# zju3dv/LoFTR

Hardware: AMD Instinct MI355X
Metric: image-pairs/sec @640x480 indoor-ds (higher is better)
Workload: dtype f32; 1 GPU; batch=8 640x480 synthetic grayscale pairs per GPU, indoor_ds dual-softmax (BASELINE configs[1]), full LoFTR.forward = ResNet-FPN backbone (HIP implicit-GEMM / patch convolutions incl. the 7x7 stem) + HIP matching path; weights=seeded random init (no checkpoint on the box), conf_matrix_materialised=True, match_type=dual_softmax, global_batch=8, parallelism=dp1 (pairs sharded; RCCL all-gather of match counts)

## Files before the change

loftr_amd/csrc/common.h:

```cpp
#pragma once
#include <hip/hip_runtime.h>
#include <stdint.h>
#include <stddef.h>
#include "../../include/loftr_hip.h"

typedef float f32x16 __attribute__((ext_vector_type(16)));
typedef float f32x4 __attribute__((ext_vector_type(4)));
typedef float f32x2 __attribute__((ext_vector_type(2)));

#define LOFTR_NEG_INF (-1e9f)

#define LOFTR_CHECK_ARG(cond) do { if (!(cond)) return LOFTR_ERR_BAD_ARG; } while (0)
#define LOFTR_CHECK_LAUNCH() do { if (hipGetLastError() != hipSuccess) return LOFTR_ERR_LAUNCH; } while (0)

#ifdef __HIP_DEVICE_COMPILE__
#define LOFTR_NO_PACKED_FP32 __attribute__((target("no-packed-fp32-ops")))
#else
#define LOFTR_NO_PACKED_FP32
#endif

__host__ __device__ static inline int ceil_div(int a, int b) { return (a + b - 1) / b; }
static inline size_t align_up(size_t x, size_t a) { return (x + a - 1) / a * a; }

enum LoftrTimedKernel {
  LOFTR_T_SCORE_STATS = 0,
  LOFTR_T_SCORE_CONF = 1,
  LOFTR_T_PROJ = 2,
  LOFTR_T_LINEAR = 3,
  LOFTR_T_LINEAR_LN = 4,
  LOFTR_T_KV = 5,
  LOFTR_T_ATTN_APPLY = 6,
  LOFTR_T_ATTN_SMALL = 7,
  LOFTR_T_GATHER = 8,
  LOFTR_T_OT_STORE = 9,
  LOFTR_T_CONV = 10,
  LOFTR_T_CONV3 = 11,
  LOFTR_T_CONV3W = 12,
  LOFTR_T_ENCODER_X = 13,
  LOFTR_T_FINE_PAIR = 14,
  LOFTR_T_COUNT = 15
};
enum LoftrDebugKey {
  LOFTR_DBG_ENCODER_SCHEDULE = 0,
  LOFTR_DBG_CONV_PERSIST_CAP,
  LOFTR_DBG_WGRAD_CHUNK,
  LOFTR_DBG_REDUCE_TALL,
  LOFTR_DBG_PCT_GRID,
  LOFTR_DBG_PCT_SKIP,
  LOFTR_DBG_PCT_QUOTA,
  LOFTR_DBG_CONV_DUO,
  LOFTR_DBG_CONV_PATCH,
  LOFTR_DBG_CONV_REM,
  LOFTR_DBG_FINE_WAVES,
  LOFTR_DBG_COUNT
};
int loftr_debug_value(int key);
extern unsigned g_loftr_timing_mask;
extern int g_loftr_range_check;
void loftr_timing_mark(int id, hipStream_t st, bool end);
struct TimedLaunch {
  int id; hipStream_t st; bool on;
  TimedLaunch(int id_, hipStream_t st_) : id(id_), st(st_), on((g_loftr_timing_mask >> id_) & 1u) {
    if (on) loftr_timing_mark(id, st, false);
  }
  ~TimedLaunch() { if (on) loftr_timing_mark(id, st, true); }
};

constexpr int NUM_XCD = 8;
static inline unsigned xcd_grid(int tiles_m, int tiles_n) { return (unsigned)(NUM_XCD * ceil_div(tiles_m, NUM_XCD) * tiles_n); }
__device__ __forceinline__ bool xcd_tile(int tiles_m, int tiles_n, int& tile_m, int& tile_n) {
  const int id = blockIdx.x, xcd = id % NUM_XCD, slot = id / NUM_XCD;
  const int chunk = ceil_div(tiles_m, NUM_XCD);
  tile_n = slot % tiles_n;
  const int local = slot / tiles_n;
  tile_m = xcd * chunk + local;
  return local < chunk && tile_m < tiles_m;
}

struct WsAlloc {
  char* base; size_t cap; size_t off;
  WsAlloc(void* p, size_t bytes) : base((char*)p), cap(bytes), off(0) {}
  template <typename T> T* take(size_t n) {
    off = align_up(off, 256);
    T* r = (T*)(base + off);
    off += n * sizeof(T);
    return r;
  }
  bool ok() const { return off <= cap; }
};

__device__ __forceinline__ float wave_sum(float v) {
#pragma unroll
  for (int o = 32; o >= 1; o >>= 1) v += __shfl_xor(v, o, 64);
  return v;
}
__device__ __forceinline__ float wave_max(float v) {
#pragma unroll
  for (int o = 32; o >= 1; o >>= 1) v = fmaxf(v, __shfl_xor(v, o, 64));
  return v;
}
#define LOFTR_DPP(v_, ctrl_) __int_as_float(__builtin_amdgcn_update_dpp(0, __float_as_int(v_), ctrl_, 0xF, 0xF, true))
#define LOFTR_DPPI(v_, ctrl_) __builtin_amdgcn_update_dpp(0, v_, ctrl_, 0xF, 0xF, true)
__device__ __forceinline__ float half_sum(float v) {
  v += LOFTR_DPP(v, 0xB1);
  v += LOFTR_DPP(v, 0x4E);
  v += LOFTR_DPP(v, 0x141);
  v += LOFTR_DPP(v, 0x140);
  const auto r = __builtin_amdgcn_permlane16_swap(__float_as_int(v), __float_as_int(v), false, false);
  return __int_as_float(r[0]) + __int_as_float(r[1]);
}
__device__ __forceinline__ float half_max(float v) {
  v = fmaxf(v, LOFTR_DPP(v, 0xB1));
  v = fmaxf(v, LOFTR_DPP(v, 0x4E));
  v = fmaxf(v, LOFTR_DPP(v, 0x141));
  v = fmaxf(v, LOFTR_DPP(v, 0x140));
  const auto r = __builtin_amdgcn_permlane16_swap(__float_as_int(v), __float_as_int(v), false, false);
  return fmaxf(__int_as_float(r[0]), __int_as_float(r[1]));
}
__device__ __forceinline__ int half_min_i32(int v) {
  v = min(v, LOFTR_DPPI(v, 0xB1));
  v = min(v, LOFTR_DPPI(v, 0x4E));
  v = min(v, LOFTR_DPPI(v, 0x141));
  v = min(v, LOFTR_DPPI(v, 0x140));
  const auto r = __builtin_amdgcn_permlane16_swap(v, v, false, false);
  return min((int)r[0], (int)r[1]);
}
__device__ __forceinline__ void half_sum16(f32x16& v) {
#pragma unroll
  for (int r = 0; r < 16; ++r) v[r] += LOFTR_DPP(v[r], 0xB1);
#pragma unroll
  for (int r = 0; r < 16; ++r) v[r] += LOFTR_DPP(v[r], 0x4E);
#pragma unroll
  for (int r = 0; r < 16; ++r) v[r] += LOFTR_DPP(v[r], 0x141);
#pragma unroll
  for (int r = 0; r < 16; ++r) v[r] += LOFTR_DPP(v[r], 0x140);
#pragma unroll
// ... 30 lines not shown
```

loftr_amd/csrc/conv.hip:

```cpp
#include "gemm.h"
#include "conv_prepared.h"
#include <stdlib.h>

namespace {

using CfgD = GemmCfg<256, 128, 4, 2, 3>;

struct ConvArgs {
  ASrc a;
  const sp_t* w; int K;
  const float* bias;
  const float* wscale;
  const float* x_inv;
  const sp_t* residual;
  sp_t* y_sp;
  float* y_f32;
  int M, Cout, Coutp;
  int act;
  const sp_t* up;
  int Hl, Wl;
  float sy, sx;
};

template <typename Cfg, bool FULL>
__device__ __forceinline__ void conv_epilogue(const ConvArgs& p, f32x16 (&acc)[Cfg::TM][Cfg::TN], int m0, int n0) {
  const EpiLane<Cfg> e;
  const sp_t* rs = p.residual ? p.residual + (long)m0 * p.Coutp + n0 : nullptr;
  sp_t* os = p.y_sp ? p.y_sp + (long)m0 * p.Coutp + n0 : nullptr;
  float* of = p.y_f32 ? p.y_f32 + (long)m0 * p.Cout + n0 : nullptr;
#pragma unroll
  for (int j = 0; j < Cfg::TN; ++j) {
    const int col = n0 + e.lcol + j * 32;
    const bool creal = col < p.Cout;
    const bool cpad = col < p.Coutp;
    const float b = (p.bias && creal) ? p.bias[col] : 0.f;
    const float wsc = (creal ? p.wscale[col] : 1.f) * (p.x_inv ? *p.x_inv : 1.f);
#pragma unroll
    for (int i = 0; i < Cfg::TM; ++i) {
      f32x16 v = acc[i][j] * wsc;
      if (rs) {
        uint32_t w[16];
#pragma unroll
        for (int r = 0; r < 16; ++r) {
          const int trow = e.lrow + e.rr(i, r);
          const bool ok = (FULL || m0 + trow < p.M) && cpad;
          w[r] = ok ? rs[(unsigned)(trow * p.Coutp + e.spcol + j * 32)] : 0u;
        }
#pragma unroll
        for (int r = 0; r < 16; ++r) v[r] += sp_value(w[r], e.odd);
      }
#pragma unroll
      for (int r = 0; r < 16; ++r) {
        float x = v[r] + b;
        if (p.act == 1) x = fmaxf(x, 0.f);
        if (p.act == 2) x = x > 0.f ? x : 0.01f * x;
        v[r] = creal ? x : 0.f;
      }
      if (of) {
#pragma unroll
        for (int r = 0; r < 16; ++r) {
          const int trow = e.lrow + e.rr(i, r);
          if ((FULL || m0 + trow < p.M) && creal) of[(unsigned)(trow * p.Cout + e.lcol + j * 32)] = v[r];
        }
      }
      if (os) {
        uint32_t w[16];
        sp_words16(v, e.odd, w);
#pragma unroll
        for (int r = 0; r < 16; ++r) {
          const int trow = e.lrow + e.rr(i, r);
          if ((FULL || m0 + trow < p.M) && cpad) os[(unsigned)(trow * p.Coutp + e.spcol + j * 32)] = w[r];
        }
      }
    }
  }
}

template <typename Cfg>
__device__ __forceinline__ void conv_epilogue_up(const ConvArgs& p, f32x16 (&acc)[Cfg::TM][Cfg::TN], int m0, int n0,
                                                 float* lds) {
  constexpr int LD = Cfg::BN + 4;
  static_assert(Cfg::BM * LD <= Cfg::LDS_FLOATS, "accumulator tile does not fit the operand ring");
  const EpiLane<Cfg> e;
  __syncthreads();
  const float xinv = p.x_inv ? *p.x_inv : 1.f;
#pragma unroll
  for (int j = 0; j < Cfg::TN; ++j) {
    const int col = n0 + e.lcol + j * 32;
    const float wsc = (col < p.Cout ? p.wscale[col] : 1.f) * xinv;
#pragma unroll
    for (int i = 0; i < Cfg::TM; ++i)
#pragma unroll
      for (int r = 0; r < 16; ++r) lds[(e.lrow + e.rr(i, r)) * LD + e.lcol + j * 32] = acc[i][j][r] * wsc;
  }
  __syncthreads();
  const int Wo = 2 * p.Wl, Ho = 2 * p.Hl;
  constexpr int OCTS = Cfg::BN / 8;
  for (int it = threadIdx.x; it < Cfg::BM * OCTS; it += Cfg::THREADS) {
    const int row = it / OCTS, oct = it - row * OCTS;
    const int pix = m0 + row, col0 = n0 + oct * 8;
    if (pix >= p.M || col0 >= p.Coutp) continue;
    const int t = pix / Wo, x = pix - t * Wo;
    const int bb = t / Ho, y = t - bb * Ho;
    const float fy = p.sy * (float)y, fx = p.sx * (float)x;
    const int y0 = (int)fy, x0 = (int)fx;
    const int dy = y0 < p.Hl - 1 ? p.Wl * p.Coutp : 0, dx = x0 < p.Wl - 1 ? p.Coutp : 0;
    const float ly = fy - (float)y0, lx = fx - (float)x0;
    const float hy = 1.f - ly, hx = 1.f - lx;
    const int off = sp_octet_off(col0 >> 3);
    const sp_t* s00 = p.up + (unsigned)(((bb * p.Hl + y0) * p.Wl + x0) * p.Coutp + off);
    const sp_t* src[4] = {s00, s00 + dx, s00 + dy, s00 + dy + dx};
    u32x4 hi[4], lo[4];
#pragma unroll
    for (int k = 0; k < 4; ++k) {
      hi[k] = *reinterpret_cast<const u32x4*>(src[k]);
      lo[k] = *reinterpret_cast<const u32x4*>(src[k] + 16);
    }
    float v[4][8], o[8];
#pragma unroll
    for (int k = 0; k < 4; ++k) sp_unpack8(hi[k], lo[k], v[k]);
    const f32x4 a0 = *reinterpret_cast<const f32x4*>(&lds[row * LD + oct * 8]);
    const f32x4 a1 = *reinterpret_cast<const f32x4*>(&lds[row * LD + oct * 8 + 4]);
#pragma unroll
    for (int c = 0; c < 8; ++c)
      o[c] = col0 + c < p.Cout
                 ? (c < 4 ? a0[c] : a1[c - 4]) + (hy * (hx * v[0][c] + lx * v[1][c]) + ly * (hx * v[2][c] + lx * v[3][c]))
                 : 0.f;
    u32x4 oh, ol;
    sp_pack8(o, oh, ol);
    sp_t* dst = p.y_sp + (unsigned)(pix * p.Coutp + off);
    *reinterpret_cast<u32x4*>(dst) = oh;
    *reinterpret_cast<u32x4*>(dst + 16) = ol;
  }
}

template <typename Cfg, bool UP>
__global__ __launch_bounds__(Cfg::THREADS, 2) void conv_kernel(ConvArgs p) {
  __shared__ __attribute__((aligned(16))) float lds[Cfg::LDS_FLOATS];
  int tm, tn;
  if (!xcd_tile(ceil_div(p.M, Cfg::BM), ceil_div(p.Coutp, Cfg::BN), tm, tn)) return;
  const int m0 = tm * Cfg::BM, n0 = tn * Cfg::BN;
  f32x16 acc[Cfg::TM][Cfg::TN];
  gemm_mainloop<Cfg, true>(p.a, p.w, p.K, p.M, p.Cout, p.K, m0, n0, lds, acc, p.Coutp);
  if constexpr (UP) conv_epilogue_up<Cfg>(p, acc, m0, n0, lds);
  else if (m0 + Cfg::BM <= p.M) conv_epilogue<Cfg, true>(p, acc, m0, n0);
  else conv_epilogue<Cfg, false>(p, acc, m0, n0);
}

namespace c3 {
constexpr int TY = 8, TX = 32, PW = TX + 2, PH = TY + 2, PROWS = PW * PH;
constexpr int PSLOTS = 43, PQ = 6;
constexpr int PATCH_BYTES = PSLOTS * 1024, BTILE_BYTES = 128 * 128;
constexpr int NB = 4;
constexpr int LDS_BYTES = 2 * PATCH_BYTES + NB * BTILE_BYTES + 1024;
using Cfg = GemmCfg<256, 128, 4, 2, 3>;
}

struct Conv3Args {
  const sp_t* x; int B, H, W, Cp, Cin;
  const sp_t* w; int K;
  const float* bias; const float* wscale; const float* x_inv; const sp_t* residual; sp_t* y_sp; float* y_f32;
  int Cout, Coutp, act;
  const sp_t* zeros;
  int tiles_x, tiles_y;
  float* pbuf;
};

__global__ __launch_bounds__(512, 2) void conv3x3_kernel(Conv3Args p) {
  using namespace c3;
  typedef __attribute__((address_space(3))) void* lds_ptr_t;
  typedef const __attribute__((address_space(1))) void* gbl_ptr_t;
  __shared__ __attribute__((aligned(16))) char lds[LDS_BYTES];
  char* const patch_base = lds;
  char* const bring_base = lds + 2 * PATCH_BYTES;
  char* const scratch = lds + 2 * PATCH_BYTES + NB * BTILE_BYTES;

  const int tid = threadIdx.x, lane = tid & 63, wave = tid >> 6;
  const int wm = wave & 3, wn = wave >> 2;
  const int rsub = lane >> 3, slot = lane & 7;

  const int tiles_m = p.B * p.tiles_y * p.tiles_x, tiles_n = ceil_div(p.Coutp, 128);
  const int chunk_m = ceil_div(tiles_m, NUM_XCD), nvirt = NUM_XCD * chunk_m * tiles_n;
  int vid = blockIdx.x;
  int nb = 0, ny0 = 0, nx0 = 0, nn0 = 0;
  bool have = false;
#define C3_NEXT_TILE()                                                                                      \
  {                                                                                                         \
    have = false;                                                                                           \
    for (; vid < nvirt; vid += gridDim.x) {                                                                 \
      const int xcd__ = vid % NUM_XCD, slot__ = vid / NUM_XCD;                                              \
      const int local__ = slot__ / tiles_n, tm__ = xcd__ * chunk_m + local__;                               \
      if (local__ < chunk_m && tm__ < tiles_m) {                                                            \
        nb = tm__ / (p.tiles_y * p.tiles_x);                                                                \
        const int trem__ = tm__ - nb * (p.tiles_y * p.tiles_x);                                             \
        ny0 = (trem__ / p.tiles_x) * TY; nx0 = (trem__ % p.tiles_x) * TX; nn0 = (slot__ % tiles_n) * 128;   \
        have = true;                                                                                        \
        break;                                                                                              \
      }                                                                                                     \
    }                                                                                                       \
  }
  C3_NEXT_TILE()
  if (!have) return;

  int poff[PQ];
  int boff[2];
#define C3_DMA_OFFSETS()                                                                                    \
  {                                                                                                         \
    _Pragma("unroll") for (int q = 0; q < PQ; ++q) {                                                        \
      const int s = q * 8 + wave, r = s * 8 + rsub;                                                         \
      const int py = r / PW, px = r - py * PW;                                                              \
      const int gy = ny0 - 1 + py, gx = nx0 - 1 + px;                                                       \
      const bool in = s < PSLOTS && r < PROWS && (unsigned)gy < (unsigned)p.H && (unsigned)gx < (unsigned)p.W; \
      poff[q] = in ? ((nb * p.H + gy) * p.W + gx) * p.Cp + ((slot ^ ((r >> 1) & 7)) << 2) : -1;             \
    }                                                                                                       \
    _Pragma("unroll") for (int q = 0; q < 2; ++q) {                                                         \
      const int r = (q * 8 + wave) * 8 + rsub;                                                              \
      boff[q] = min(nn0 + r, p.Cout - 1) * p.K + ((slot ^ ((r >> 1) & 7)) << 2);                            \
    }                                                                                                       \
  }
  C3_DMA_OFFSETS()
// ... 230 lines not shown
  const int co = blockIdx.x;
  float scale = 1.f, shift = 0.f;
  if (bn_w) {
    scale = bn_w[co] / sqrtf(bn_v[co] + eps);
    shift = bn_b[co] - bn_m[co] * scale;
  }
  float m = 0.f;
  for (int t = threadIdx.x; t < Cin * KH * KW; t += 256) {
    const int c = t % Cin, tap = t / Cin;
    m = fmaxf(m, fabsf(w[co * s_co + c * s_ci + (tap / KW) * s_ky + (tap % KW) * s_kx] * scale));
  }
  __shared__ float red[4];
  m = wave_max(m);
  if ((threadIdx.x & 63) == 0) red[threadIdx.x >> 6] = m;
  __syncthreads();
  if (threadIdx.x == 0) {
    float inv;
    (void)sp_row_scale(fmaxf(fmaxf(red[0], red[1]), fmaxf(red[2], red[3])), &inv);
    bias[co] = shift;
    wscale[co] = inv;
  }
}

__global__ __launch_bounds__(256) void conv_prep_kernel(const float* __restrict__ w, const float* __restrict__ bn_w,
                                                        const float* __restrict__ bn_b, const float* __restrict__ bn_m,
                                                        const float* __restrict__ bn_v, float eps, int Cin, int Cp,
                                                        int KH, int KW, long s_co, long s_ci, long s_ky, long s_kx,
                                                        sp_t* __restrict__ wsp, const float* __restrict__ wscale) {
  const int co = blockIdx.y;
  const int K = KH * KW * Cp;
  float scale = 1.f;
  if (bn_w) scale = bn_w[co] / sqrtf(bn_v[co] + eps);
  const float up = 1.f / wscale[co];
  const int grp = blockIdx.x * 8 + (threadIdx.x >> 5);
  if (grp * 32 >= K) return;
  const int col = grp * 32 + (threadIdx.x & 31);
  const int tap = col / Cp, c = col - tap * Cp;
  float v = 0.f;
  if (c < Cin) v = (w[co * s_co + c * s_ci + (tap / KW) * s_ky + (tap % KW) * s_kx] * scale) * up;
  sp_store(wsp + (long)co * K, col, v, true);
}

__global__ __launch_bounds__(256) void upsample_add_kernel(const sp_t* __restrict__ low, const sp_t* __restrict__ lat,
                                                           sp_t* __restrict__ out, int Hl, int Wl, int Cp, long nitems) {
  const long item = (long)blockIdx.x * 256 + threadIdx.x;
  if (item >= nitems) return;
  const int octs = Cp >> 3;
  const long pix = item / octs;
  const int oct = (int)(item - pix * octs);
  const int Ho = 2 * Hl, Wo = 2 * Wl;
  const int x = (int)(pix % Wo), y = (int)((pix / Wo) % Ho);
  const long b = pix / ((long)Wo * Ho);
  const float sy = Ho > 1 ? (float)(Hl - 1) / (float)(Ho - 1) : 0.f, sx = Wo > 1 ? (float)(Wl - 1) / (float)(Wo - 1) : 0.f;
  const float fy = sy * (float)y, fx = sx * (float)x;
  const int y0 = (int)fy, x0 = (int)fx;
  const int y1 = y0 + (y0 < Hl - 1 ? 1 : 0), x1 = x0 + (x0 < Wl - 1 ? 1 : 0);
  const float ly = fy - (float)y0, lx = fx - (float)x0;
  const float hy = 1.f - ly, hx = 1.f - lx;
  const int off = sp_octet_off(oct);
  const sp_t* src[5] = {low + ((b * Hl + y0) * Wl + x0) * Cp + off, low + ((b * Hl + y0) * Wl + x1) * Cp + off,
                        low + ((b * Hl + y1) * Wl + x0) * Cp + off, low + ((b * Hl + y1) * Wl + x1) * Cp + off,
                        lat + pix * Cp + off};
  u32x4 hi[5], lo[5];
#pragma unroll
  for (int t = 0; t < 5; ++t) {
    hi[t] = *reinterpret_cast<const u32x4*>(src[t]);
    lo[t] = *reinterpret_cast<const u32x4*>(src[t] + 16);
  }
  float v[5][8];
#pragma unroll
  for (int t = 0; t < 5; ++t) sp_unpack8(hi[t], lo[t], v[t]);
  float r[8];
#pragma unroll
  for (int e = 0; e < 8; ++e)
    r[e] = v[4][e] + (hy * (hx * v[0][e] + lx * v[1][e]) + ly * (hx * v[2][e] + lx * v[3][e]));
  u32x4 oh, ol;
  sp_pack8(r, oh, ol);
  sp_t* o = out + pix * Cp + off;
  *reinterpret_cast<u32x4*>(o) = oh;
  *reinterpret_cast<u32x4*>(o + 16) = ol;
}

constexpr int STEM_TY = 8, STEM_TX = 32;
__global__ __launch_bounds__(256) void stem_conv_kernel(const float* __restrict__ x, long sxb, long sxh, long sxw,
                                                        int H, int W, const float* __restrict__ w, long s_co, long s_ky,
                                                        long s_kx, const float* __restrict__ bn_w,
                                                        const float* __restrict__ bn_b, const float* __restrict__ bn_m,
                                                        const float* __restrict__ bn_v, float eps, int C0, int Ho, int Wo,
                                                        sp_t* __restrict__ y) {
  constexpr int IH = 2 * STEM_TY + 5, IW = 2 * STEM_TX + 5;
  __shared__ float tile[IH][IW + 3];
  const int b = blockIdx.z, oy0 = blockIdx.y * STEM_TY, ox0 = blockIdx.x * STEM_TX;
  const float* xb = x + (long)b * sxb;
  for (int e = threadIdx.x; e < IH * IW; e += 256) {
    const int r = e / IW, c = e - r * IW;
    const int iy = 2 * oy0 - 3 + r, ix = 2 * ox0 - 3 + c;
    tile[r][c] = ((unsigned)iy < (unsigned)H && (unsigned)ix < (unsigned)W) ? xb[iy * sxh + ix * sxw] : 0.f;
  }
  const int ch = threadIdx.x & 127, slot = threadIdx.x >> 7;
  float wr[49];
  float scale = 1.f, shift = 0.f;
  if (ch < C0) {
    if (bn_w) { scale = bn_w[ch] / sqrtf(bn_v[ch] + eps); shift = bn_b[ch] - bn_m[ch] * scale; }
#pragma unroll
    for (int t = 0; t < 49; ++t) wr[t] = w[ch * s_co + (t / 7) * s_ky + (t % 7) * s_kx] * scale;
  } else {
#pragma unroll
    for (int t = 0; t < 49; ++t) wr[t] = 0.f;
  }
  __syncthreads();
  const int Cp = (C0 + 31) / 32 * 32;
  for (int q = slot; q < STEM_TY * STEM_TX / 4; q += 2) {
    const int py = q / (STEM_TX / 4), px = (q - py * (STEM_TX / 4)) * 4;
    float acc[4] = {shift, shift, shift, shift};
#pragma unroll
    for (int ky = 0; ky < 7; ++ky) {
      float row[13];
#pragma unroll
      for (int c = 0; c < 13; ++c) row[c] = tile[2 * py + ky][2 * px + c];
#pragma unroll
      for (int kx = 0; kx < 7; ++kx)
#pragma unroll
        for (int e = 0; e < 4; ++e) acc[e] += row[2 * e + kx] * wr[ky * 7 + kx];
    }
    const int oy = oy0 + py;
#pragma unroll
    for (int e = 0; e < 4; ++e) {
      const int ox = ox0 + px + e;
      const float v = fmaxf(acc[e], 0.f);
      const bool ok = oy < Ho && ox < Wo && ch < Cp;
      const uint32_t word = sp_word(ch < C0 ? v : 0.f, ch & 1);
      if (ok) y[(((long)b * Ho + oy) * Wo + ox) * Cp + sp_index(ch)] = word;
    }
  }
}

__global__ void sp_to_f32_kernel(const sp_t* __restrict__ src, float* __restrict__ dst, long rows, int C, int Cp) {
  const long row = blockIdx.x;
  for (int c = threadIdx.x; c < Cp; c += blockDim.x) {
    const float v = sp_value(src[row * Cp + sp_index(c)], c & 1);
    if (c < C) dst[row * C + c] = v;
  }
}

}

extern "C" size_t loftr_conv_workspace_bytes(int Cin, int Cout, int KH, int KW) {
  if (Cin <= 0 || Cout <= 0 || KH <= 0 || KW <= 0) return 0;
  return align_up((size_t)Cout * KH * KW * ceil32(Cin) * 4, 256) + 2 * align_up((size_t)Cout * 4, 256) + 2048;
}

static unsigned persistent_grid(unsigned nvirt) {
  const int cap = loftr_debug_value(LOFTR_DBG_CONV_PERSIST_CAP);
  const int forced = cap >= NUM_XCD ? cap / NUM_XCD * NUM_XCD : -1;
  int cus = forced;
  if (cus < 0) {
    static int per_dev[64];
    int dev = 0, n = 0;
    if (hipGetDevice(&dev) != hipSuccess || dev < 0 || dev >= 64) return nvirt;
    if (per_dev[dev] == 0) {
      if (hipDeviceGetAttribute(&n, hipDeviceAttributeMultiprocessorCount, dev) != hipSuccess) return nvirt;
      per_dev[dev] = n / NUM_XCD * NUM_XCD;
    }
    cus = per_dev[dev];
  }
  return cus > 0 && nvirt > (unsigned)cus ? (unsigned)cus : nvirt;
}

template <int RT>
__global__ __launch_bounds__(256) void conv_rem_gather_kernel(const float* __restrict__ pbuf, long npix, int H, int W, int R, int c0, int Coutp,
                                                              const float* __restrict__ bias, const sp_t* __restrict__ residual, int act,
                                                              sp_t* __restrict__ y_sp) {
  const long pix = (long)blockIdx.x * 256 + threadIdx.x;
  if (pix >= npix) return;
  const int x = (int)(pix % W), y = (int)((pix / W) % H);
  float v[8];
#pragma unroll
  for (int c = 0; c < 8; ++c) v[c] = 0.f;
  const float* pp = pbuf + pix * (9 * R);
#pragma unroll
  for (int ky = 0; ky < 3; ++ky)
#pragma unroll
    for (int kx = 0; kx < 3; ++kx) {
      const int yy = y + ky - 1, xx = x + kx - 1;
      if ((unsigned)yy < (unsigned)H && (unsigned)xx < (unsigned)W) {
        const float* q = pp + ((long)(ky - 1) * W + (kx - 1)) * (9 * R) + (ky * 3 + kx) * R;
        if (RT == 4) {
          const f32x4 t = *reinterpret_cast<const f32x4*>(q);
          v[0] += t[0]; v[1] += t[1]; v[2] += t[2]; v[3] += t[3];
        } else {
#pragma unroll
          for (int c = 0; c < 7; ++c) if (c < R) v[c] += q[c];
        }
      }
    }
  sp_t* row = y_sp + pix * Coutp + c0;
  float rv[8];
#pragma unroll
  for (int c = 0; c < 8; ++c) rv[c] = 0.f;
  if (residual) {
    const sp_t* rr = residual + pix * Coutp + c0;
    const u32x4 hi = *reinterpret_cast<const u32x4*>(rr), lo = *reinterpret_cast<const u32x4*>(rr + 16);
    sp_unpack8(hi, lo, rv);
  }
  const float slope = act == 1 ? 0.f : act == 2 ? 0.01f : 1.f;
  float o[8];
#pragma unroll
  for (int c = 0; c < 8; ++c) {
    const float t = v[c] + ((bias && c < R) ? bias[c0 + c] : 0.f) + rv[c];
    o[c] = c < R ? fmaxf(t, slope * t) : 0.f;
  }
  u32x4 oh, ol;
  sp_pack8(o, oh, ol);
  const u32x4 z = {0u, 0u, 0u, 0u};
  u32x4* dst = reinterpret_cast<u32x4*>(row);
  dst[0] = oh; dst[1] = z; dst[2] = z; dst[3] = z; dst[4] = ol; dst[5] = z; dst[6] = z; dst[7] = z;
}


static int conv_prepare(const float* weight, const long* weight_strides, int Cin, int Cout, int KH, int KW,
                        const float* bn_weight, const float* bn_bias, const float* bn_mean, const float* bn_var, float bn_eps,
                        void* buf, size_t bytes, hipStream_t st) {
  LOFTR_CHECK_ARG(weight && weight_strides && buf && Cin > 0 && Cout > 0 && KH > 0 && KW > 0);
  LOFTR_CHECK_ARG((bn_weight == nullptr) == (bn_bias == nullptr) && (bn_weight == nullptr) == (bn_mean == nullptr) &&
                  (bn_weight == nullptr) == (bn_var == nullptr));
  ConvPrepared pr;
  if (!conv_prepared_layout(buf, bytes, Cin, Cout, KH, KW, pr)) return LOFTR_ERR_WORKSPACE;
  const int Cp = ceil32(Cin), K = KH * KW * Cp;
  (void)hipMemsetAsync(pr.zeros, 0, 256, st);
  hipLaunchKernelGGL(conv_rowscale_kernel, dim3(Cout), dim3(256), 0, st, weight, bn_weight, bn_bias, bn_mean, bn_var, bn_eps,
                     Cin, KH, KW, weight_strides[0], weight_strides[1], weight_strides[2], weight_strides[3], pr.bias, pr.wscale);
  hipLaunchKernelGGL(conv_prep_kernel, dim3(ceil_div(K / 32, 8), Cout), dim3(256), 0, st, weight, bn_weight, bn_bias,
                     bn_mean, bn_var, bn_eps, Cin, Cp, KH, KW, weight_strides[0], weight_strides[1], weight_strides[2],
                     weight_strides[3], pr.wsp, pr.wscale);
  LOFTR_CHECK_LAUNCH();
  return LOFTR_OK;
}

static int conv_rem_channels(int Cout, int KH, int KW, int stride) {
  return (KH == 3 && KW == 3 && stride == 1 && ceil32(Cout) == 224 && Cout - 192 >= 1 && Cout - 192 <= 7) ? Cout - 192 : 0;
}
extern "C" size_t loftr_conv_scratch_bytes(int B, int H, int W, int Cout, int KH, int KW, int stride) {
  const int R = conv_rem_channels(Cout, KH, KW, stride);
  return (R > 0 && B > 0 && H > 0 && W > 0) ? (size_t)B * H * W * 9 * R * 4 : 0;
}

static int conv_run(const uint32_t* x_sp, int B, int H, int W, int Cin, const void* prepared, size_t prepared_bytes, int Cout,
                    int KH, int KW, int stride, int pad, int act, const uint32_t* residual_sp, const uint32_t* up_sp,
                    uint32_t* y_sp, float* y_f32, void* stream, const float* x_inv = nullptr, void* scratch = nullptr, size_t scratch_bytes = 0) {
  LOFTR_CHECK_ARG(x_sp && prepared && (y_sp || y_f32) && B >= 0 && H > 0 && W > 0 && Cin > 0 && Cout > 0);
  const bool shared_gpu = (act & LOFTR_CONV_SHARED_GPU) != 0;
  act &= ~LOFTR_CONV_SHARED_GPU;
  LOFTR_CHECK_ARG(KH > 0 && KW > 0 && stride > 0 && pad >= 0 && act >= 0 && act <= 2);
  if (B == 0) return LOFTR_OK;
  hipStream_t st = (hipStream_t)stream;
  ConvGeom g;
  g.H = H; g.W = W; g.Cp = ceil32(Cin); g.KH = KH; g.KW = KW; g.stride = stride; g.pad = pad;
  g.Ho = (H + 2 * pad - KH) / stride + 1;
  g.Wo = (W + 2 * pad - KW) / stride + 1;
  if (g.Ho <= 0 || g.Wo <= 0 || H >= 32768 || W >= 32768) return LOFTR_ERR_UNSUPPORTED;
  if (up_sp && ((g.Ho & 1) || (g.Wo & 1) || KH != 1 || KW != 1 || stride != 1 || pad != 0 || !y_sp || y_f32 || residual_sp || act != 0))
    return LOFTR_ERR_UNSUPPORTED;
  const long M = (long)B * g.Ho * g.Wo;
  if (M * (long)ceil32(Cout) >= (1L << 31) || (long)B * H * W * g.Cp >= (1L << 31)) return LOFTR_ERR_UNSUPPORTED;
  const int K = KH * KW * g.Cp;
  ConvPrepared pr;
  if (!conv_prepared_layout(const_cast<void*>(prepared), prepared_bytes, Cin, Cout, KH, KW, pr)) return LOFTR_ERR_WORKSPACE;
  sp_t* wsp = pr.wsp;
  float* bias = pr.bias;
  sp_t* zeros = pr.zeros;
  g.zeros = zeros;
  ConvArgs p;
  p.a = asrc_conv(x_sp, g);
  p.w = wsp; p.K = K; p.bias = bias; p.wscale = pr.wscale; p.x_inv = x_inv; p.residual = residual_sp; p.y_sp = y_sp; p.y_f32 = y_f32;
  p.M = (int)M; p.Cout = Cout; p.Coutp = ceil32(Cout); p.act = act;
  p.up = up_sp; p.Hl = g.Ho / 2; p.Wl = g.Wo / 2;
  p.sy = g.Ho > 1 ? (float)(p.Hl - 1) / (float)(g.Ho - 1) : 0.f;
  p.sx = g.Wo > 1 ? (float)(p.Wl - 1) / (float)(g.Wo - 1) : 0.f;
  if (loftr_debug_value(LOFTR_DBG_CONV_PATCH) && KH == 3 && KW == 3 && stride == 1 && pad == 1 && !up_sp) {
    Conv3Args c;
    c.x = x_sp; c.B = B; c.H = H; c.W = W; c.Cp = g.Cp; c.Cin = Cin; c.w = wsp; c.K = K; c.bias = bias; c.wscale = pr.wscale; c.x_inv = x_inv; c.residual = residual_sp;
    c.y_sp = y_sp; c.y_f32 = y_f32; c.Cout = Cout; c.Coutp = ceil32(Cout); c.act = act; c.zeros = zeros;
    c.tiles_x = ceil_div(W, c3::TX); c.tiles_y = ceil_div(H, c3::TY); c.pbuf = nullptr;
    const bool duo = loftr_debug_value(LOFTR_DBG_CONV_DUO) != 0;
    const bool wide = duo && c.Coutp == 32 * 7;
    TimedLaunch tl(wide ? LOFTR_T_CONV3W : LOFTR_T_CONV3, st);
    if (duo && c.Coutp % 128 == 0) {
      using CF = c3d::Cfg<4, 2, 4>;
      c.tiles_y = ceil_div(H, CF::TY);
      hipLaunchKernelGGL((conv3x3_duo_kernel<CF>), dim3(xcd_grid(B * c.tiles_x * c.tiles_y, c.Coutp / 128)), dim3(256), 0, st, c);
    } else if (duo && c.Coutp == 192) {
      using CF = c3d::Cfg<6, 2, 4, 8, 2>;
      c.tiles_y = ceil_div(H, CF::TY);
      hipLaunchKernelGGL((conv3x3_duo_kernel<CF>), dim3(xcd_grid(B * c.tiles_x * c.tiles_y, 1)), dim3(512), 0, st, c);
    } else if (wide && conv_rem_channels(Cout, KH, KW, stride) > 0 && !y_f32 && loftr_debug_value(LOFTR_DBG_CONV_REM) &&
               scratch && scratch_bytes >= (size_t)B * H * W * 9 * conv_rem_channels(Cout, KH, KW, stride) * 4) {
      using CF = c3d::Cfg<6, 2, 4, 8, 2, true>;
      c.tiles_y = ceil_div(H, CF::TY);
      c.pbuf = reinterpret_cast<float*>(scratch);
      hipLaunchKernelGGL((conv3x3_duo_kernel<CF>), dim3(xcd_grid(B * c.tiles_x * c.tiles_y, 1)), dim3(512), 0, st, c);
      LOFTR_CHECK_LAUNCH();
      const long npix = (long)B * H * W;
      if (Cout - 192 == 4)
        hipLaunchKernelGGL(conv_rem_gather_kernel<4>, dim3((unsigned)((npix + 255) / 256)), dim3(256), 0, st, c.pbuf, npix, H, W, 4, 192, c.Coutp,
                           bias, residual_sp, act, y_sp);
      else
        hipLaunchKernelGGL(conv_rem_gather_kernel<0>, dim3((unsigned)((npix + 255) / 256)), dim3(256), 0, st, c.pbuf, npix, H, W, Cout - 192, 192, c.Coutp,
                           bias, residual_sp, act, y_sp);
    } else if (wide) {
      using CF = c3d::Cfg<7, 2, 4, 8, 2>;
      c.tiles_y = ceil_div(H, CF::TY);
      hipLaunchKernelGGL((conv3x3_duo_kernel<CF>), dim3(xcd_grid(B * c.tiles_x * c.tiles_y, 1)), dim3(512), 0, st, c);
    } else
      hipLaunchKernelGGL(conv3x3_kernel, dim3(shared_gpu ? xcd_grid(B * c.tiles_x * c.tiles_y, ceil_div(c.Coutp, 128))
                                                         : persistent_grid(xcd_grid(B * c.tiles_x * c.tiles_y, ceil_div(c.Coutp, 128)))),
                         dim3(512), 0, st, c);
    LOFTR_CHECK_LAUNCH();
    return LOFTR_OK;
  }
  {
    TimedLaunch tl(LOFTR_T_CONV, st);
    if (up_sp)
      hipLaunchKernelGGL((conv_kernel<CfgD, true>), dim3(xcd_grid(ceil_div(p.M, CfgD::BM), ceil_div(p.Coutp, CfgD::BN))),
                         dim3(CfgD::THREADS), 0, st, p);
    else
      hipLaunchKernelGGL((conv_kernel<CfgD, false>), dim3(xcd_grid(ceil_div(p.M, CfgD::BM), ceil_div(p.Coutp, CfgD::BN))),
                         dim3(CfgD::THREADS), 0, st, p);
  }
  LOFTR_CHECK_LAUNCH();
  return LOFTR_OK;
}

#ifdef LOFTR_CONV_PROBE
extern "C" int loftr_conv_probe_buffer(void* buf) {
  long long* b = (long long*)buf;
  return hipMemcpyToSymbol(HIP_SYMBOL(g_conv_probe), &b, sizeof(b)) == hipSuccess ? LOFTR_OK : LOFTR_ERR_LAUNCH;
}
#endif

extern "C" int loftr_conv_prepare(const float* weight, const long* weight_strides, int Cin, int Cout, int KH, int KW,
                                  const float* bn_weight, const float* bn_bias, const float* bn_mean, const float* bn_var,
                                  float bn_eps, void* prepared, size_t prepared_bytes, void* stream) {
  return conv_prepare(weight, weight_strides, Cin, Cout, KH, KW, bn_weight, bn_bias, bn_mean, bn_var, bn_eps, prepared,
                      prepared_bytes, (hipStream_t)stream);
}

extern "C" int loftr_conv_bn_act_prepared(const uint32_t* x_sp, int B, int H, int W, int Cin, const void* prepared,
                                          size_t prepared_bytes, int Cout, int KH, int KW, int stride, int pad, int act,
                                          const uint32_t* residual_sp, const uint32_t* low_sp, uint32_t* y_sp, float* y_f32,
                                          const float* x_inv_scale, void* stream) {
  return conv_run(x_sp, B, H, W, Cin, prepared, prepared_bytes, Cout, KH, KW, stride, pad, act, residual_sp, low_sp, y_sp, y_f32,
                  stream, x_inv_scale);
}

extern "C" int loftr_conv_bn_act_prepared_scratch(const uint32_t* x_sp, int B, int H, int W, int Cin, const void* prepared,
                                                  size_t prepared_bytes, int Cout, int KH, int KW, int stride, int pad, int act,
                                                  const uint32_t* residual_sp, const uint32_t* low_sp, uint32_t* y_sp, float* y_f32,
                                                  const float* x_inv_scale, void* scratch, size_t scratch_bytes, void* stream) {
  return conv_run(x_sp, B, H, W, Cin, prepared, prepared_bytes, Cout, KH, KW, stride, pad, act, residual_sp, low_sp, y_sp, y_f32,
                  stream, x_inv_scale, scratch, scratch_bytes);
}

extern "C" int loftr_conv_bn_act(const uint32_t* x_sp, int B, int H, int W, int Cin, const float* weight,
                                 const long* weight_strides, int Cout, int KH, int KW, int stride, int pad, const float* bn_weight, const float* bn_bias,
                                 const float* bn_mean, const float* bn_var, float bn_eps, int act,
                                 const uint32_t* residual_sp, uint32_t* y_sp, float* y_f32, void* ws, size_t ws_bytes,
                                 const float* x_inv_scale, void* stream) {
  LOFTR_CHECK_ARG(x_sp && (y_sp || y_f32) && B >= 0 && H > 0 && W > 0);
  if (B == 0) return LOFTR_OK;
  const int rc = conv_prepare(weight, weight_strides, Cin, Cout, KH, KW, bn_weight, bn_bias, bn_mean, bn_var, bn_eps, ws, ws_bytes,
                              (hipStream_t)stream);
  if (rc != LOFTR_OK) return rc;
  return conv_run(x_sp, B, H, W, Cin, ws, ws_bytes, Cout, KH, KW, stride, pad, act, residual_sp, nullptr, y_sp, y_f32, stream, x_inv_scale);
}

extern "C" int loftr_conv1x1_upsample_add(const uint32_t* x_sp, int B, int H, int W, int Cin, const float* weight,
                                          const long* weight_strides, int Cout, const uint32_t* low_sp, uint32_t* y_sp,
                                          void* ws, size_t ws_bytes, void* stream) {
  LOFTR_CHECK_ARG(x_sp && low_sp && y_sp && B >= 0 && H > 0 && W > 0);
  if (B == 0) return LOFTR_OK;
  const int rc = conv_prepare(weight, weight_strides, Cin, Cout, 1, 1, nullptr, nullptr, nullptr, nullptr, 0.f, ws, ws_bytes,
                              (hipStream_t)stream);
  if (rc != LOFTR_OK) return rc;
  return conv_run(x_sp, B, H, W, Cin, ws, ws_bytes, Cout, 1, 1, 1, 0, 0, nullptr, low_sp, y_sp, nullptr, stream);
}

extern "C" int loftr_stem_conv_bn_relu(const float* x, const long* x_strides, int B, int H, int W, const float* weight,
                                       const long* weight_strides, int C0, const float* bn_weight, const float* bn_bias,
                                       const float* bn_mean, const float* bn_var, float bn_eps, uint32_t* y_sp,
                                       void* stream) {
  LOFTR_CHECK_ARG(x && x_strides && weight && weight_strides && y_sp && B >= 0 && H > 0 && W > 0 && C0 > 0);
  LOFTR_CHECK_ARG((bn_weight == nullptr) == (bn_bias == nullptr) && (bn_weight == nullptr) == (bn_mean == nullptr) &&
                  (bn_weight == nullptr) == (bn_var == nullptr));
  if (C0 > 128) return LOFTR_ERR_UNSUPPORTED;
  if (B == 0) return LOFTR_OK;
  const int Ho = (H + 6 - 7) / 2 + 1, Wo = (W + 6 - 7) / 2 + 1;
  hipLaunchKernelGGL(stem_conv_kernel, dim3(ceil_div(Wo, STEM_TX), ceil_div(Ho, STEM_TY), B), dim3(256), 0,
                     (hipStream_t)stream, x, x_strides[0], x_strides[2], x_strides[3], H, W, weight, weight_strides[0],
                     weight_strides[2], weight_strides[3], bn_weight, bn_bias, bn_mean, bn_var, bn_eps, C0, Ho, Wo, y_sp);
  LOFTR_CHECK_LAUNCH();
  return LOFTR_OK;
}

extern "C" int loftr_upsample2x_add(const uint32_t* low_sp, const uint32_t* lateral_sp, uint32_t* out_sp, int B, int Hl,
                                    int Wl, int C, void* stream) {
  LOFTR_CHECK_ARG(low_sp && lateral_sp && out_sp && B >= 0 && Hl > 0 && Wl > 0 && C > 0);
  if (B == 0) return LOFTR_OK;
  const int Cp = ceil32(C);
  const long pixels = (long)B * 4 * Hl * Wl;
  if (pixels >= (1L << 31)) return LOFTR_ERR_UNSUPPORTED;
  const long nitems = pixels * (Cp / 8);
  if ((nitems + 255) / 256 >= (1L << 31)) return LOFTR_ERR_UNSUPPORTED;
  hipLaunchKernelGGL(upsample_add_kernel, dim3((unsigned)((nitems + 255) / 256)), dim3(256), 0, (hipStream_t)stream,
                     low_sp, lateral_sp, out_sp, Hl, Wl, Cp, nitems);
  LOFTR_CHECK_LAUNCH();
  return LOFTR_OK;
}

extern "C" int loftr_sp_from_f32(const float* src, uint32_t* dst_sp, long rows, int C, void* stream) {
  LOFTR_CHECK_ARG(src && dst_sp && rows >= 0 && C > 0);
  return launch_sp_convert1(src, C, dst_sp, rows, C, (hipStream_t)stream);
}

extern "C" int loftr_sp_from_f32_scaled(const float* src, uint32_t* dst_sp, long rows, int C, float* inv_scale_out, void* stream) {
  LOFTR_CHECK_ARG(src && dst_sp && inv_scale_out && rows >= 0 && C > 0);
  return launch_sp_convert1(src, C, dst_sp, rows, C, (hipStream_t)stream, inv_scale_out);
}

extern "C" int loftr_sp_to_f32(const uint32_t* src_sp, float* dst, long rows, int C, void* stream) {
  LOFTR_CHECK_ARG(src_sp && dst && rows >= 0 && C > 0);
  if (rows == 0) return LOFTR_OK;
  const int Cp = ceil32(C);
  hipLaunchKernelGGL(sp_to_f32_kernel, dim3((unsigned)rows), dim3(Cp > 256 ? 256 : Cp), 0, (hipStream_t)stream, src_sp,
                     dst, rows, C, Cp);
  LOFTR_CHECK_LAUNCH();
  return LOFTR_OK;
}
```

loftr_amd/csrc/misc.hip:

```cpp
#include "common.h"
#include <string.h>

namespace {
template <bool CL>
__global__ void pos_encode_flatten_kernel(loftr_fmap f, const float* __restrict__ pe,
                                          int pe_h, int pe_w, float* __restrict__ out, int C) {
  __shared__ float tile[32][33];
  const int H = f.H, W = f.W, HW = H * W;
  const int n = blockIdx.z, hw0 = blockIdx.x * 32, c0 = blockIdx.y * 32;
  const float* in = f.data + (long)n * f.sn;
  for (int k = threadIdx.y; k < 32; k += 8) {
    const int c = c0 + k, hw = hw0 + threadIdx.x;
    float v = 0.f;
    if (c < C && hw < HW) {
      const int y = hw / W, x = hw - y * W;
      v = pe[((long)c * pe_h + y) * pe_w + x];
      if (!CL) v += in[(long)c * f.sc + (long)y * f.sh + (long)x * f.sw];
    }
    tile[k][threadIdx.x] = v;
  }
  __syncthreads();
  for (int k = threadIdx.y; k < 32; k += 8) {
    const int hw = hw0 + k, c = c0 + threadIdx.x;
    if (hw < HW && c < C) {
      float v = tile[threadIdx.x][k];
      if (CL) { const int y = hw / W, x = hw - y * W; v += in[(long)y * f.sh + (long)x * f.sw + c]; }
      out[((long)n * HW + hw) * C + c] = v;
    }
  }
}
}

extern "C" int loftr_pos_encode_flatten(const loftr_fmap* feat, const float* pe, int pe_h, int pe_w, float* out,
                                        int N, int C, void* stream) {
  LOFTR_CHECK_ARG(feat && feat->data && pe && out && N >= 0 && C > 0 && feat->H > 0 && feat->W > 0 &&
                  feat->H <= pe_h && feat->W <= pe_w);
  if (N == 0) return LOFTR_OK;
  const dim3 grid(ceil_div(feat->H * feat->W, 32), ceil_div(C, 32), N), block(32, 8);
  if (feat->sc == 1)
    hipLaunchKernelGGL((pos_encode_flatten_kernel<true>), grid, block, 0, (hipStream_t)stream, *feat, pe, pe_h, pe_w, out, C);
  else
    hipLaunchKernelGGL((pos_encode_flatten_kernel<false>), grid, block, 0, (hipStream_t)stream, *feat, pe, pe_h, pe_w, out, C);
  LOFTR_CHECK_LAUNCH();
  return LOFTR_OK;
}

namespace {
struct DebugSwitch { const char* name; int def; int value; };
DebugSwitch g_debug[LOFTR_DBG_COUNT] = {{"encoder_schedule", 1, 1}, {"conv_persist_cap", 0, 0}, {"wgrad_chunk", 0, 0}, {"reduce_tall", 1, 1},
                                        {"pct_grid", 0, 0}, {"pct_skip", 0, 0}, {"pct_quota", 0, 0}, {"conv_duo", 1, 1}, {"conv_patch", 1, 1}, {"conv_rem", 1, 1},
                                        {"fine_waves", 0, 0}};
}
int loftr_debug_value(int key) { return (key >= 0 && key < LOFTR_DBG_COUNT) ? g_debug[key].value : 0; }
extern "C" int loftr_hip_debug_set(const char* key, int value) {
  LOFTR_CHECK_ARG(key != nullptr);
  for (auto& d : g_debug)
    if (strcmp(d.name, key) == 0) { d.value = value; return LOFTR_OK; }
  return LOFTR_ERR_BAD_ARG;
}
extern "C" int loftr_hip_debug_get(const char* key, int* value, int* default_value) {
  LOFTR_CHECK_ARG(key != nullptr && value != nullptr);
  for (auto& d : g_debug)
    if (strcmp(d.name, key) == 0) { *value = d.value; if (default_value) *default_value = d.def; return LOFTR_OK; }
  return LOFTR_ERR_BAD_ARG;
}

unsigned g_loftr_timing_mask = 0;
int g_loftr_range_check = 0;
extern "C" int loftr_hip_range_check_enable(int on) { g_loftr_range_check = on ? 1 : 0; return LOFTR_OK; }
namespace {
constexpr int T_POOL = 4096;
struct TimingSlot {
  hipEvent_t ev[T_POOL][2];
  int created, used;
  double total_ms; long long launches;
};
TimingSlot g_slots[LOFTR_T_COUNT];
const char* const T_NAMES[LOFTR_T_COUNT] = {"score_sweep_kernel<0>", "score_sweep_kernel<1>", "proj_kernel", "linear_kernel",
                                            "linear_ln_kernel", "proj_kv_kernel", "attn_apply_kernel",
                                            "attn_small_kernel", "gather_windows_kernel", "score_sweep_kernel<2>", "conv_kernel",
                                            "conv3x3_duo_kernel<Cfg<4,2,4,4,1>>", "conv3x3_duo_kernel<Cfg<7,2,4,8,2>>", "encoder_x_kernel", "fine_pair_kernel"};
void timing_drain(TimingSlot& s) {
  for (int i = 0; i < s.used; ++i) {
    float ms = 0.f;
    if (hipEventSynchronize(s.ev[i][1]) == hipSuccess && hipEventElapsedTime(&ms, s.ev[i][0], s.ev[i][1]) == hipSuccess) {
      s.total_ms += ms;
      s.launches += 1;
    }
  }
  s.used = 0;
}
}

void loftr_timing_mark(int id, hipStream_t st, bool end) {
  TimingSlot& s = g_slots[id];
  if (!end) {
    if (s.used >= T_POOL) return;
    if (s.used >= s.created) {
      if (hipEventCreate(&s.ev[s.created][0]) != hipSuccess || hipEventCreate(&s.ev[s.created][1]) != hipSuccess) return;
      s.created++;
    }
    (void)hipEventRecord(s.ev[s.used][0], st);
  } else {
    if (s.used >= s.created) return;
    (void)hipEventRecord(s.ev[s.used][1], st);
    s.used++;
  }
}

extern "C" int loftr_hip_timing_enable(unsigned mask) {
  g_loftr_timing_mask = mask & ((1u << LOFTR_T_COUNT) - 1u);
  return LOFTR_OK;
}

extern "C" int loftr_hip_timing_kernel_count(void) { return LOFTR_T_COUNT; }

extern "C" const char* loftr_hip_timing_kernel_name(int id) {
  return (id >= 0 && id < LOFTR_T_COUNT) ? T_NAMES[id] : "";
}

extern "C" int loftr_hip_timing_read(int id, double* total_ms, long long* launches, int reset) {
  LOFTR_CHECK_ARG(id >= 0 && id < LOFTR_T_COUNT && total_ms && launches);
  TimingSlot& s = g_slots[id];
  timing_drain(s);
  *total_ms = s.total_ms;
  *launches = s.launches;
  if (reset) { s.total_ms = 0.0; s.launches = 0; }
  return LOFTR_OK;
}

extern "C" int loftr_hip_abi_version(void) { return LOFTR_HIP_ABI_VERSION; }

extern "C" const char* loftr_hip_status_string(int status) {
  switch (status) {
// ... 20 lines not shown
```

Baseline: 445.5 image-pairs/s.

## Add packed-FMA stem conv and single-pass wide-N conv tile for 224/256 channels

Adds a new 7x7 stem convolution body that stores the input tile as even/odd column planes and computes two output pixels per packed v_pk_fma_f32, with each thread producing a 4x4 output block. Separately, for convolutions whose padded output width is 224 or 256, a 256x256 GEMM tile covering all output channels in one pass is launched when a CU-occupancy heuristic favours it, with launch bounds relaxed to one workgroup per SIMD. Both are on by default behind debug switches. The wider tile raises register pressure and lowers occupancy in exchange for reading the A operand only once.

```diff
diff --git a/loftr_amd/csrc/common.h b/loftr_amd/csrc/common.h
--- a/loftr_amd/csrc/common.h
+++ b/loftr_amd/csrc/common.h
@@ -52,6 +52,8 @@
   LOFTR_DBG_CONV_PATCH,
   LOFTR_DBG_CONV_REM,
   LOFTR_DBG_FINE_WAVES,
+  LOFTR_DBG_STEM_PACKED,
+  LOFTR_DBG_CONV_ONEPASS,
   LOFTR_DBG_COUNT
 };
 int loftr_debug_value(int key);
diff --git a/loftr_amd/csrc/conv.hip b/loftr_amd/csrc/conv.hip
--- a/loftr_amd/csrc/conv.hip
+++ b/loftr_amd/csrc/conv.hip
@@ -5,6 +5,7 @@
 namespace {
 
 using CfgD = GemmCfg<256, 128, 4, 2, 3>;
+using CfgW = GemmCfg<256, 256, 4, 2, 2>;
 
 struct ConvArgs {
   ASrc a;
@@ -135,7 +136,7 @@
 }
 
 template <typename Cfg, bool UP>
-__global__ __launch_bounds__(Cfg::THREADS, 2) void conv_kernel(ConvArgs p) {
+__global__ __launch_bounds__(Cfg::THREADS, Cfg::TM * Cfg::TN > 4 ? 1 : 2) void conv_kernel(ConvArgs p) {
   __shared__ __attribute__((aligned(16))) float lds[Cfg::LDS_FLOATS];
   int tm, tn;
   if (!xcd_tile(ceil_div(p.M, Cfg::BM), ceil_div(p.Coutp, Cfg::BN), tm, tn)) return;
@@ -532,7 +533,7 @@
 }
 
 constexpr int STEM_TY = 8, STEM_TX = 32;
-__global__ __launch_bounds__(256) void stem_conv_kernel(const float* __restrict__ x, long sxb, long sxh, long sxw,
+__device__ __forceinline__ void stem_body(const float* __restrict__ x, long sxb, long sxh, long sxw,
                                                         int H, int W, const float* __restrict__ w, long s_co, long s_ky,
                                                         long s_kx, const float* __restrict__ bn_w,
                                                         const float* __restrict__ bn_b, const float* __restrict__ bn_m,
@@ -583,6 +584,124 @@
       if (ok) y[(((long)b * Ho + oy) * Wo + ox) * Cp + sp_index(ch)] = word;
     }
   }
+}
+
+typedef float stem_f32x2 __attribute__((ext_vector_type(2)));
+typedef float stem_f32x4 __attribute__((ext_vector_type(4)));
+template <int HI>
+__device__ __forceinline__ void stem_pk_fma(stem_f32x2& acc, stem_f32x2 w, stem_f32x2 r) {
+  if constexpr (HI) asm("v_pk_fma_f32 %0, %1, %2, %0 op_sel:[1,0,0] op_sel_hi:[1,1,1]" : "+v"(acc) : "v"(w), "v"(r));
+  else asm("v_pk_fma_f32 %0, %1, %2, %0 op_sel:[0,0,0] op_sel_hi:[0,1,1]" : "+v"(acc) : "v"(w), "v"(r));
+}
+template <int KY, int KX>
+__device__ __forceinline__ void stem_pk_taps(stem_f32x2& a01, stem_f32x2& a23, const stem_f32x2 (&w2)[25],
+                                             const stem_f32x2 (&ep)[6], const stem_f32x2 (&op)[5]) {
+  if constexpr (KX < 7) {
+    constexpr int t = KY * 7 + KX, j = KX / 2;
+    if constexpr (KX % 2 == 0) {
+      stem_pk_fma<t & 1>(a01, w2[t / 2], ep[j]);
+      stem_pk_fma<t & 1>(a23, w2[t / 2], ep[j + 2]);
+    } else {
+      stem_pk_fma<t & 1>(a01, w2[t / 2], op[j]);
+      stem_pk_fma<t & 1>(a23, w2[t / 2], op[j + 2]);
+    }
+    stem_pk_taps<KY, KX + 1>(a01, a23, w2, ep, op);
+  }
+}
+constexpr int STEM_PLANE = 40;
+constexpr int STEM_BR = 4;
+template <int R, int J>
+__device__ __forceinline__ void stem_pk_feed(stem_f32x2 (&a)[STEM_BR][2], const stem_f32x2 (&w2)[25], const stem_f32x2 (&ep)[6],
+                                             const stem_f32x2 (&op)[5]) {
+  if constexpr (J < STEM_BR) {
+    if constexpr (R - 2 * J >= 0 && R - 2 * J < 7) stem_pk_taps<R - 2 * J, 0>(a[J][0], a[J][1], w2, ep, op);
+    stem_pk_feed<R, J + 1>(a, w2, ep, op);
+  }
+}
+typedef stem_f32x2 __attribute__((aligned(4))) stem_f32x2_u;
+template <int R>
+__device__ __forceinline__ void stem_pk_rows(stem_f32x2 (&a)[STEM_BR][2], const stem_f32x2 (&w2)[25], const float* t0, const float* t1) {
+  if constexpr (R < 2 * STEM_BR + 5) {
+    const float* e = t0 + R * 2 * STEM_PLANE;
+    const float* o = e + STEM_PLANE;
+    const float* es = t1 + R * 2 * STEM_PLANE;
+    const float* os = es + STEM_PLANE;
+    const stem_f32x4 e03 = *reinterpret_cast<const stem_f32x4*>(e), o03 = *reinterpret_cast<const stem_f32x4*>(o);
+    const stem_f32x2 ep[6] = {{e03.x, e03.y}, *reinterpret_cast<const stem_f32x2_u*>(es), {e03.z, e03.w},
+                              *reinterpret_cast<const stem_f32x2_u*>(es + 2), *reinterpret_cast<const stem_f32x2*>(e + 4),
+                              *reinterpret_cast<const stem_f32x2_u*>(es + 4)};
+    const stem_f32x2 op[5] = {{o03.x, o03.y}, *reinterpret_cast<const stem_f32x2_u*>(os), {o03.z, o03.w},
+                              *reinterpret_cast<const stem_f32x2_u*>(os + 2), *reinterpret_cast<const stem_f32x2*>(o + 4)};
+    stem_pk_feed<R, 0>(a, w2, ep, op);
+    stem_pk_rows<R + 1>(a, w2, t0, t1);
+  }
+}
+__device__ __forceinline__ void stem_body_pk(const float* __restrict__ x, long sxb, long sxh, long sxw,
+                                                           int H, int W, const float* __restrict__ w, long s_co, long s_ky,
+                                                           long s_kx, const float* __restrict__ bn_w,
+                                                           const float* __restrict__ bn_b, const float* __restrict__ bn_m,
+                                                           const float* __restrict__ bn_v, float eps, int C0, int Ho, int Wo,
+                                                           sp_t* __restrict__ y) {
+  constexpr int IH = 2 * STEM_TY + 5, IW = 2 * STEM_TX + 5;
+  static_assert((IW + 1) / 2 <= STEM_PLANE && STEM_TX - 4 + 6 < (IW + 1) / 2 && STEM_TX - 4 + 5 < IW / 2, "window row fits its planes");
+  __shared__ __attribute__((aligned(16))) float tile[IH][2 * STEM_PLANE];
+  const int b = blockIdx.z, oy0 = blockIdx.y * STEM_TY, ox0 = blockIdx.x * STEM_TX;
+  const float* xb = x + (long)b * sxb;
+  for (int e = threadIdx.x; e < IH * IW; e += 256) {
+    const int r = e / IW, c = e - r * IW;
+    const int iy = 2 * oy0 - 3 + r, ix = 2 * ox0 - 3 + c;
+    tile[r][(c & 1) * STEM_PLANE + (c >> 1)] = ((unsigned)iy < (unsigned)H && (unsigned)ix < (unsigned)W) ? xb[iy * sxh + ix * sxw] : 0.f;
+  }
+  const int ch = threadIdx.x & 127, slot = threadIdx.x >> 7;
+  stem_f32x2 w2[25];
+  float scale = 1.f, shift = 0.f;
+  if (ch < C0) {
+    if (bn_w) { scale = bn_w[ch] / sqrtf(bn_v[ch] + eps); shift = bn_b[ch] - bn_m[ch] * scale; }
+#pragma unroll
+    for (int t = 0; t < 49; ++t) {
+      const float v = w[ch * s_co + (t / 7) * s_ky + (t % 7) * s_kx] * scale;
+      if (t & 1) w2[t / 2].y = v; else w2[t / 2].x = v;
+    }
+    w2[24].y = 0.f;
+  } else {
+#pragma unroll
+    for (int t = 0; t < 25; ++t) w2[t] = stem_f32x2{0.f, 0.f};
+  }
+  __syncthreads();
+  const int Cp = (C0 + 31) / 32 * 32;
+  int one = 1;
+  asm("" : "+v"(one));
+  static_assert(STEM_TY % STEM_BR == 0 && STEM_TX % 4 == 0, "blocks tile the workgroup's patch");
+  for (int q = slot; q < (STEM_TY / STEM_BR) * (STEM_TX / 4); q += 2) {
+    const int by = q / (STEM_TX / 4), px = (q - by * (STEM_TX / 4)) * 4;
+    stem_f32x2 a[STEM_BR][2];
+#pragma unroll
+    for (int j = 0; j < STEM_BR; ++j) a[j][0] = a[j][1] = stem_f32x2{shift, shift};
+    const float* t0 = &tile[2 * STEM_BR * by][px];
+    stem_pk_rows<0>(a, w2, t0, t0 + one);
+#pragma unroll
+    for (int j = 0; j < STEM_BR; ++j) {
+      const float acc[4] = {a[j][0].x, a[j][0].y, a[j][1].x, a[j][1].y};
+      const int oy = oy0 + STEM_BR * by + j;
+#pragma unroll
+      for (int e = 0; e < 4; ++e) {
+        const int ox = ox0 + px + e;
+        const float v = fmaxf(acc[e], 0.f);
+        const bool ok = oy < Ho && ox < Wo && ch < Cp;
+        const uint32_t word = sp_word(ch < C0 ? v : 0.f, ch & 1);
+        if (ok) y[(((long)b * Ho + oy) * Wo + ox) * Cp + sp_index(ch)] = word;
+      }
+    }
+  }
+}
+template <bool PACKED>
+__global__ __launch_bounds__(256) void stem_conv_kernel(const float* __restrict__ x, long sxb, long sxh, long sxw, int H, int W,
+                                                        const float* __restrict__ w, long s_co, long s_ky, long s_kx,
+                                                        const float* __restrict__ bn_w, const float* __restrict__ bn_b,
+                                                        const float* __restrict__ bn_m, const float* __restrict__ bn_v, float eps,
+                                                        int C0, int Ho, int Wo, sp_t* __restrict__ y) {
+  if constexpr (PACKED) stem_body_pk(x, sxb, sxh, sxw, H, W, w, s_co, s_ky, s_kx, bn_w, bn_b, bn_m, bn_v, eps, C0, Ho, Wo, y);
+  else stem_body(x, sxb, sxh, sxw, H, W, w, s_co, s_ky, s_kx, bn_w, bn_b, bn_m, bn_v, eps, C0, Ho, Wo, y);
 }
 
 __global__ void sp_to_f32_kernel(const sp_t* __restrict__ src, float* __restrict__ dst, long rows, int C, int Cp) {
@@ -693,6 +812,13 @@
 extern "C" size_t loftr_conv_scratch_bytes(int B, int H, int W, int Cout, int KH, int KW, int stride) {
   const int R = conv_rem_channels(Cout, KH, KW, stride);
   return (R > 0 && B > 0 && H > 0 && W > 0) ? (size_t)B * H * W * 9 * R * 4 : 0;
+}
+
+static bool conv_onepass_pays(int row_tiles) {
+  const int mode = loftr_debug_value(LOFTR_DBG_CONV_ONEPASS);
+  if (mode != 1) return mode != 0;
+  const int cus = (int)persistent_grid(1u << 30);
+  return 5 * ceil_div(row_tiles, cus) <= 3 * ceil_div(2 * row_tiles, cus);
 }
 
 static int conv_run(const uint32_t* x_sp, int B, int H, int W, int Cin, const void* prepared, size_t prepared_bytes, int Cout,
@@ -773,6 +899,8 @@
     if (up_sp)
       hipLaunchKernelGGL((conv_kernel<CfgD, true>), dim3(xcd_grid(ceil_div(p.M, CfgD::BM), ceil_div(p.Coutp, CfgD::BN))),
                          dim3(CfgD::THREADS), 0, st, p);
+    else if ((p.Coutp == 224 || p.Coutp == 256) && conv_onepass_pays(ceil_div(p.M, CfgW::BM)))
+      hipLaunchKernelGGL((conv_kernel<CfgW, false>), dim3(xcd_grid(ceil_div(p.M, CfgW::BM), 1)), dim3(CfgW::THREADS), 0, st, p);
     else
       hipLaunchKernelGGL((conv_kernel<CfgD, false>), dim3(xcd_grid(ceil_div(p.M, CfgD::BM), ceil_div(p.Coutp, CfgD::BN))),
                          dim3(CfgD::THREADS), 0, st, p);
@@ -845,7 +973,8 @@
   if (C0 > 128) return LOFTR_ERR_UNSUPPORTED;
   if (B == 0) return LOFTR_OK;
   const int Ho = (H + 6 - 7) / 2 + 1, Wo = (W + 6 - 7) / 2 + 1;
-  hipLaunchKernelGGL(stem_conv_kernel, dim3(ceil_div(Wo, STEM_TX), ceil_div(Ho, STEM_TY), B), dim3(256), 0,
+  const auto kernel = loftr_debug_value(LOFTR_DBG_STEM_PACKED) ? stem_conv_kernel<true> : stem_conv_kernel<false>;
+  hipLaunchKernelGGL(kernel, dim3(ceil_div(Wo, STEM_TX), ceil_div(Ho, STEM_TY), B), dim3(256), 0,
                      (hipStream_t)stream, x, x_strides[0], x_strides[2], x_strides[3], H, W, weight, weight_strides[0],
                      weight_strides[2], weight_strides[3], bn_weight, bn_bias, bn_mean, bn_var, bn_eps, C0, Ho, Wo, y_sp);
   LOFTR_CHECK_LAUNCH();
diff --git a/loftr_amd/csrc/misc.hip b/loftr_amd/csrc/misc.hip
--- a/loftr_amd/csrc/misc.hip
+++ b/loftr_amd/csrc/misc.hip
@@ -49,7 +49,7 @@
 struct DebugSwitch { const char* name; int def; int value; };
 DebugSwitch g_debug[LOFTR_DBG_COUNT] = {{"encoder_schedule", 1, 1}, {"conv_persist_cap", 0, 0}, {"wgrad_chunk", 0, 0}, {"reduce_tall", 1, 1},
                                         {"pct_grid", 0, 0}, {"pct_skip", 0, 0}, {"pct_quota", 0, 0}, {"conv_duo", 1, 1}, {"conv_patch", 1, 1}, {"conv_rem", 1, 1},
-                                        {"fine_waves", 0, 0}};
+                                        {"fine_waves", 0, 0}, {"stem_packed", 1, 1}, {"conv_onepass", 1, 1}};
 }
 int loftr_debug_value(int key) { return (key >= 0 && key < LOFTR_DBG_COUNT) ? g_debug[key].value : 0; }
 extern "C" int loftr_hip_debug_set(const char* key, int value) {
```

Result: no change. 449.6 image-pairs/s, median of 6 (+0.9%).
